# foolwood/SiamMask

Hardware: NVIDIA H100
Metric: search-region frames/sec (127/255 SiamMask-sharp) (higher is better)
Workload: dtype f16x3 (hi+lo split fp16 operands on wgmma, f32 accumulate; f32 CUDA-core xcorr/refine)

## Files before the change

### siammask_b200/csrc/common.cuh

```cuda
#pragma once
#include <cuda.h>
#include <cuda_fp16.h>
#include <cuda_runtime.h>
#include <cstdint>
#include <cstdio>
#include <stdexcept>
#include <string>
#include <vector>

namespace smk {

struct Act {
  __half* hi = nullptr;
  __half* lo = nullptr;
  int B = 0, H = 0, W = 0, C = 0;
  int sexp = 0;
  __host__ __device__ size_t numel() const { return (size_t)B * H * W * C; }
  __host__ __device__ int M() const { return B * H * W; }
};

struct ConvGeom {
  int Cin, Cout, KH, KW, stride, pad, dil;
  __host__ __device__ int out_size(int in) const { return (in + 2 * pad - dil * (KH - 1) - 1) / stride + 1; }
};

enum OutMode : int { OUT_NHWC_SPLIT = 0, OUT_NHWC_F32 = 1, OUT_NCHW_F32 = 2 };

struct Epilogue {
  const float* alpha = nullptr;
  const float* beta = nullptr;
  const __half* res_hi = nullptr;
  const __half* res_lo = nullptr;
  __half* out_hi = nullptr;
  __half* out_lo = nullptr;
  float* out_f32 = nullptr;
  int out_mode = OUT_NHWC_SPLIT;
  int relu = 0;
  int* ovf = nullptr;
};

__device__ __forceinline__ void flag_if_out_of_range(float absmax, int* ovf) {
  if (ovf != nullptr && !(absmax <= 65504.f)) atomicOr(ovf, 1);
}

struct GemmSegment {
  CUtensorMap tmA[2];
  int kind;
  int mode;
  int num_kb, cblks, KW;
  int stride, pad, dil;
  int b_col0;
};

struct GemmParams {
  GemmSegment seg[2];
  int nseg;
  CUtensorMap tmB[2];
  int M, Cout, Ho, Wo;
  int n_tiles, m_tiles;
  int reverse_m;
  Epilogue ep;
};

struct GemmInput {
  Act in;
  ConvGeom g;
  int w_col0;
};

struct TrackerHp {
  double context_amount, penalty_k, window_influence, lr;
  int32_t exemplar_size, instance_size, total_stride, base_size, out_size, reserved;
};

struct CudaError : std::runtime_error {
  using std::runtime_error::runtime_error;
};

#define SMK_CUDA(expr)                                                                              \
  do {                                                                                              \
    cudaError_t _e = (expr);                                                                        \
    if (_e != cudaSuccess)                                                                          \
      throw smk::CudaError(std::string(#expr) + " failed: " + cudaGetErrorString(_e) + " at " +    \
                           __FILE__ + ":" + std::to_string(__LINE__));                              \
  } while (0)

#define SMK_CHECK(cond, msg)                                                                        \
  do {                                                                                              \
    if (!(cond)) throw std::runtime_error(std::string("check failed: ") + #cond + " — " + (msg));   \
  } while (0)

template <typename K>
inline void ensure_dynamic_smem(K kernel, int bytes, unsigned long long& done_mask) {
  int dev = 0;
  SMK_CUDA(cudaGetDevice(&dev));
  const unsigned long long bit = 1ull << (dev & 63);
  if (done_mask & bit) return;
  SMK_CUDA(cudaFuncSetAttribute(kernel, cudaFuncAttributeMaxDynamicSharedMemorySize, bytes));
  done_mask |= bit;
}


bool gemm_conv_supported(const ConvGeom& g);
void launch_gemm_conv(const Act& in, const ConvGeom& g, const __half* w_hi, const __half* w_lo, int cout_pad,
                      const Epilogue& ep, int nsplit, int num_sms, cudaStream_t st);
void launch_gemm_multi(const GemmInput* convs, int nconv, const Act* residual, int res_col0, const __half* w_hi,
                       const __half* w_lo, int cout_pad, int w_ld, const Epilogue& ep, int nsplit, int num_sms,
                       cudaStream_t st, bool reverse_m = false);

CUtensorMap make_map_tiled_nd(const __half* base, int rank, const uint64_t* dims, const uint64_t* strides_bytes,
                              const uint32_t* box, int swizzle_bytes);

int patch_conv_mode();
// ... 47 lines not shown
```

### siammask_b200/csrc/conv_gemm_sm90.cu

```cuda
#include "common.cuh"
#include "ptx.cuh"

#include <cstdlib>
#include <cstring>
#include <mutex>
#include <unordered_map>

namespace smk {

namespace {

constexpr int BLOCK_M = 128;
constexpr int BLOCK_K = 64;
constexpr int CIN_GRAIN = 64;
constexpr int MMA_K = 16;
constexpr int SMEM_LIMIT = 227 * 1024;
constexpr int NUM_CONSUMER_WARPS = 8;
constexpr int NUM_THREADS = 128 + 32 * NUM_CONSUMER_WARPS;
constexpr int PRODUCER_REGS = 40;
constexpr int CONSUMER_REGS = 232;

template <int BLOCK_N, int NSPLIT>
struct Cfg {
  static constexpr int A_TILE_BYTES = BLOCK_M * BLOCK_K * 2;
  static constexpr int B_TILE_BYTES = BLOCK_N * BLOCK_K * 2;
  static constexpr int STAGE_BYTES = NSPLIT * (A_TILE_BYTES + B_TILE_BYTES);
  static constexpr int RAW_STAGES = (SMEM_LIMIT - 2048) / STAGE_BYTES;
  static constexpr int STAGES = RAW_STAGES > 6 ? 6 : RAW_STAGES;
  static constexpr int SMEM_BYTES = STAGES * STAGE_BYTES + 1024  + 256 ;
  static constexpr int ACC = BLOCK_N / 2;
  static_assert(STAGES >= 2, "pipeline needs at least two stages");
  static_assert(BLOCK_N % 16 == 0 && BLOCK_N >= 16 && BLOCK_N <= 128, "N tile (register accumulators)");
  static_assert(B_TILE_BYTES % 1024 == 0, "stage parts stay 1024-aligned (swizzle atoms)");
  static_assert(SMEM_BYTES <= SMEM_LIMIT, "shared memory budget");
};

__device__ __forceinline__ int m_block(const GemmParams& p, int tile) {
  const int mb = tile / p.n_tiles;
  return p.reverse_m ? p.m_tiles - 1 - mb : mb;
}

template <int BLOCK_N, int NSPLIT>
__global__ void __launch_bounds__(NUM_THREADS, 1) conv_gemm_kernel(const __grid_constant__ GemmParams p) {
  using C = Cfg<BLOCK_N, NSPLIT>;
  constexpr int STAGES = C::STAGES;
  constexpr int A_TILE_BYTES = C::A_TILE_BYTES;

  extern __shared__ uint8_t smem_raw[];
  uint8_t* smem = reinterpret_cast<uint8_t*>((reinterpret_cast<uintptr_t>(smem_raw) + 1023) & ~uintptr_t(1023));
  uint64_t* full_bar = reinterpret_cast<uint64_t*>(smem + STAGES * C::STAGE_BYTES);
  uint64_t* empty_bar = full_bar + STAGES;

  const int warp = __shfl_sync(0xffffffffu, (int)(threadIdx.x >> 5), 0);
  const int lane = threadIdx.x & 31;
  const int num_tiles = p.m_tiles * p.n_tiles;

  if (threadIdx.x == 0) {
    for (int i = 0; i < NSPLIT; ++i) {
      for (int sgi = 0; sgi < p.nseg; ++sgi) tma_prefetch_desc(&p.seg[sgi].tmA[i]);
      tma_prefetch_desc(&p.tmB[i]);
    }
    for (int s = 0; s < STAGES; ++s) {
      mbar_init(&full_bar[s], 1);
      mbar_init(&empty_bar[s], NUM_CONSUMER_WARPS);
    }
    fence_barrier_init();
  }
  __syncthreads();

  if (warp < 4) {
    setmaxnreg_dec<PRODUCER_REGS>();
    if (warp != 0) return;
    const bool leader = elect_one();
    int stage = 0;
    uint32_t phase = 0;
    auto acquire = [&](uint32_t bytes) {
      mbar_wait(&empty_bar[stage], phase ^ 1);
      if (leader) mbar_arrive_expect_tx(&full_bar[stage], bytes);
    };
    auto load_2d = [&](void* dst, const CUtensorMap* map, int c0, int c1) {
      if (leader) tma_load_2d(dst, map, &full_bar[stage], c0, c1);
    };
    for (int tile = blockIdx.x; tile < num_tiles; tile += gridDim.x) {
      const int m0 = m_block(p, tile) * BLOCK_M;
      const int n0 = (tile % p.n_tiles) * BLOCK_N;
      const int q = m0 % p.Wo;
      const int t = m0 / p.Wo;
      const int pq = t % p.Ho;
      const int nb = t / p.Ho;
      for (int sgi = 0; sgi < p.nseg; ++sgi) {
        const GemmSegment& sg = p.seg[sgi];
        if (sg.kind == 1) {
#pragma unroll 1
          for (int kb = 0; kb < BLOCK_N / BLOCK_K; ++kb) {
            acquire(C::STAGE_BYTES);
            uint8_t* st = smem + stage * C::STAGE_BYTES;
#pragma unroll
            for (int s = 0; s < NSPLIT; ++s) {
              load_2d(st + s * A_TILE_BYTES, &sg.tmA[s], n0 + kb * BLOCK_K, m0);
              load_2d(st + NSPLIT * A_TILE_BYTES + s * C::B_TILE_BYTES, &p.tmB[s], sg.b_col0 + n0 + kb * BLOCK_K, n0);
            }
            __syncwarp();
            if (++stage == STAGES) { stage = 0; phase ^= 1; }
          }
          continue;
        }
        const int wb = q * sg.stride - sg.pad;
        const int hb = pq * sg.stride - sg.pad;
#pragma unroll 1
        for (int kb = 0; kb < sg.num_kb; ++kb) {
          acquire(C::STAGE_BYTES);
          uint8_t* st = smem + stage * C::STAGE_BYTES;
          const int tap = kb / sg.cblks;
          const int c0 = (kb - tap * sg.cblks) * BLOCK_K;
#pragma unroll
          for (int s = 0; s < NSPLIT; ++s) {
            uint8_t* a_dst = st + s * A_TILE_BYTES;
            if (sg.mode == 0) {
              load_2d(a_dst, &sg.tmA[s], c0, m0);
            } else if (leader) {
              const int r = tap / sg.KW;
              const int sx = tap - r * sg.KW;
              tma_load_im2col_4d(a_dst, &sg.tmA[s], &full_bar[stage], c0, wb, hb, nb,
                                 static_cast<uint16_t>(sx * sg.dil), static_cast<uint16_t>(r * sg.dil));
            }
            load_2d(st + NSPLIT * A_TILE_BYTES + s * C::B_TILE_BYTES, &p.tmB[s], sg.b_col0 + kb * BLOCK_K, n0);
          }
          __syncwarp();
          if (++stage == STAGES) { stage = 0; phase ^= 1; }
        }
      }
    }
    return;
  }

  setmaxnreg_inc<CONSUMER_REGS>();
  const int wg = (warp >> 2) - 1;
  const int wl = warp & 3;
  const Epilogue& ep = p.ep;
  const int HoWo = p.Ho * p.Wo;
  float acc[C::ACC];
  float acc2[C::ACC];
  int stage = 0;
  uint32_t phase = 0;
  for (int tile = blockIdx.x; tile < num_tiles; tile += gridDim.x) {
#pragma unroll
    for (int i = 0; i < C::ACC; ++i) { acc[i] = 0.f; acc2[i] = 0.f; }
    int prev = -1;
    for (int sgi = 0; sgi < p.nseg; ++sgi) {
      const GemmSegment& sg = p.seg[sgi];
      const bool ident = sg.kind == 1;
      const int nkb = ident ? BLOCK_N / BLOCK_K : sg.num_kb;
#pragma unroll 1
      for (int kb = 0; kb < nkb; ++kb) {
        mbar_wait(&full_bar[stage], phase);
        const uint32_t a_hi = smem_u32(smem + stage * C::STAGE_BYTES) + wg * (64 * BLOCK_K * 2);
        const uint32_t b_hi = smem_u32(smem + stage * C::STAGE_BYTES) + NSPLIT * A_TILE_BYTES;
        const uint64_t da_hi0 = wgmma_desc_kmajor<128>(a_hi);
        const uint64_t db_hi0 = wgmma_desc_kmajor<128>(b_hi);
        const uint64_t da_lo0 = wgmma_desc_kmajor<128>(a_hi + A_TILE_BYTES);
        const uint64_t db_lo0 = wgmma_desc_kmajor<128>(b_hi + C::B_TILE_BYTES);
        wgmma_fence();
#pragma unroll
        for (int k = 0; k < BLOCK_K / MMA_K; ++k) {
          const uint64_t kadd = static_cast<uint64_t>(k * MMA_K * 2 / 16);
          wgmma_f16<BLOCK_N>(acc, da_hi0 + kadd, db_hi0 + kadd);
          if constexpr (NSPLIT == 2) {
            wgmma_f16<BLOCK_N>(acc2, da_hi0 + kadd, db_lo0 + kadd);
            wgmma_f16<BLOCK_N>(acc2, da_lo0 + kadd, db_hi0 + kadd);
          }
        }
        wgmma_commit();
        wgmma_wait<1>();
        if (prev >= 0) {
          __syncwarp();
          if (lane == 0) mbar_arrive(&empty_bar[prev]);
        }
        prev = stage;
        if (++stage == STAGES) { stage = 0; phase ^= 1; }
      }
    }
    wgmma_wait<0>();
    fence_regs(acc);
    if constexpr (NSPLIT == 2) fence_regs(acc2);
    __syncwarp();
    if (lane == 0) mbar_arrive(&empty_bar[prev]);

    const int row0 = m_block(p, tile) * BLOCK_M + wg * 64 + wl * 16 + (lane >> 2);
    const int col0 = (tile % p.n_tiles) * BLOCK_N + 2 * (lane & 3);
    float amax = 0.f;
#pragma unroll
    for (int h = 0; h < 2; ++h) {
      const int m = row0 + 8 * h;
      if (m >= p.M) continue;
      const int b = m / HoWo;
      const int hw = m - b * HoWo;
#pragma unroll
      for (int j = 0; j < BLOCK_N / 8; ++j) {
        const int n = col0 + 8 * j;
        float v0 = acc[4 * j + 2 * h], v1 = acc[4 * j + 2 * h + 1];
        if constexpr (NSPLIT == 2) {
          v0 += acc2[4 * j + 2 * h];
          v1 += acc2[4 * j + 2 * h + 1];
        }
        const float2 al = __ldg(reinterpret_cast<const float2*>(ep.alpha + n));
        const float2 be = __ldg(reinterpret_cast<const float2*>(ep.beta + n));
        v0 = fmaf(v0, al.x, be.x);
        v1 = fmaf(v1, al.y, be.y);
        const size_t off = static_cast<size_t>(m) * p.Cout + n;
        if (ep.res_hi != nullptr) {
          const float2 f = __half22float2(*reinterpret_cast<const __half2*>(ep.res_hi + off));
          v0 += f.x;
          v1 += f.y;
          if (ep.res_lo != nullptr) {
            const float2 l = __half22float2(*reinterpret_cast<const __half2*>(ep.res_lo + off));
            v0 += l.x;
            v1 += l.y;
          }
        }
        if (ep.relu) {
          v0 = fmaxf(v0, 0.f);
          v1 = fmaxf(v1, 0.f);
        }
        if (ep.out_mode == OUT_NHWC_SPLIT) {
          amax = fmaxf(amax, fmaxf(fabsf(v0), fabsf(v1)));
          const __half2 hv = __floats2half2_rn(v0, v1);
          const float2 hf = __half22float2(hv);
          *reinterpret_cast<__half2*>(ep.out_hi + off) = hv;
          if (ep.out_lo != nullptr)
            *reinterpret_cast<__half2*>(ep.out_lo + off) = __floats2half2_rn(v0 - hf.x, v1 - hf.y);
        } else if (ep.out_mode == OUT_NHWC_F32) {
          *reinterpret_cast<float2*>(ep.out_f32 + off) = make_float2(v0, v1);
        } else if (n < p.Cout) {
          float* dst = ep.out_f32 + (static_cast<size_t>(b) * p.Cout + n) * HoWo + hw;
          __stcs(dst, v0);
          if (n + 1 < p.Cout) __stcs(dst + HoWo, v1);
        }
      }
    }
    if (ep.out_mode == OUT_NHWC_SPLIT) flag_if_out_of_range(amax, ep.ovf);
  }
}

using EncodeTiledFn = CUresult (*)(CUtensorMap*, CUtensorMapDataType, cuuint32_t, void*, const cuuint64_t*,
                                   const cuuint64_t*, const cuuint32_t*, const cuuint32_t*, CUtensorMapInterleave,
                                   CUtensorMapSwizzle, CUtensorMapL2promotion, CUtensorMapFloatOOBfill);
using EncodeIm2colFn = CUresult (*)(CUtensorMap*, CUtensorMapDataType, cuuint32_t, void*, const cuuint64_t*,
                                    const cuuint64_t*, const int*, const int*, cuuint32_t, cuuint32_t,
                                    const cuuint32_t*, CUtensorMapInterleave, CUtensorMapSwizzle,
                                    CUtensorMapL2promotion, CUtensorMapFloatOOBfill);

struct DriverApi {
  EncodeTiledFn tiled = nullptr;
  EncodeIm2colFn im2col = nullptr;
  int driver_version = 0;
};

const DriverApi& driver_api() {
  static DriverApi api;
  static std::once_flag once;
  std::call_once(once, [] {
    void* fn = nullptr;
    cudaDriverEntryPointQueryResult q;
    SMK_CUDA(cudaGetDriverEntryPoint("cuTensorMapEncodeTiled", &fn, cudaEnableDefault, &q));
    SMK_CHECK(fn != nullptr && q == cudaDriverEntryPointSuccess, "cuTensorMapEncodeTiled not available");
    api.tiled = reinterpret_cast<EncodeTiledFn>(fn);
    fn = nullptr;
    SMK_CUDA(cudaGetDriverEntryPoint("cuTensorMapEncodeIm2col", &fn, cudaEnableDefault, &q));
    SMK_CHECK(fn != nullptr && q == cudaDriverEntryPointSuccess, "cuTensorMapEncodeIm2col not available");
    api.im2col = reinterpret_cast<EncodeIm2colFn>(fn);
    SMK_CUDA(cudaDriverGetVersion(&api.driver_version));
  });
  return api;
}

struct MapKey {
  uint64_t v[16];
  bool operator==(const MapKey& o) const { return std::memcmp(v, o.v, sizeof v) == 0; }
};
struct MapKeyHash {
  size_t operator()(const MapKey& k) const {
    uint64_t h = 0x9E3779B97F4A7C15ull;
    for (uint64_t x : k.v) { h ^= x + 0x9E3779B97F4A7C15ull + (h << 6) + (h >> 2); }
    return (size_t)h;
  }
};
template <typename F>
CUtensorMap cached_map(const MapKey& key, F&& encode) {
  static std::mutex mu;
  static std::unordered_map<MapKey, CUtensorMap, MapKeyHash> cache;
  static const bool off = getenv("SMB200_NO_MAP_CACHE") != nullptr;
  if (off) return encode();
  int dev = 0;
  cudaGetDevice(&dev);
  MapKey k = key;
  k.v[15] = (uint64_t)dev;
  std::lock_guard<std::mutex> lock(mu);
  auto it = cache.find(k);
  if (it != cache.end()) return it->second;
  if (cache.size() > 65536) cache.clear();
  CUtensorMap m = encode();
  cache.emplace(k, m);
  return m;
}

CUtensorMap make_map_2d_raw(const __half* base, uint64_t inner, uint64_t outer, uint32_t box_inner, uint32_t box_outer) {
  CUtensorMap m;
  cuuint64_t dims[2] = {inner, outer};
  cuuint64_t strides[1] = {inner * sizeof(__half)};
  cuuint32_t box[2] = {box_inner, box_outer};
  cuuint32_t estr[2] = {1, 1};
  const CUtensorMapSwizzle sw = box_inner == 64 ? CU_TENSOR_MAP_SWIZZLE_128B : CU_TENSOR_MAP_SWIZZLE_64B;
  CUresult r = driver_api().tiled(&m, CU_TENSOR_MAP_DATA_TYPE_FLOAT16, 2, const_cast<__half*>(base), dims, strides,
                                  box, estr, CU_TENSOR_MAP_INTERLEAVE_NONE, sw,
                                  CU_TENSOR_MAP_L2_PROMOTION_L2_256B, CU_TENSOR_MAP_FLOAT_OOB_FILL_NONE);
  SMK_CHECK(r == CUDA_SUCCESS, "cuTensorMapEncodeTiled failed, code " + std::to_string((int)r));
  return m;
}

CUtensorMap make_map_2d(const __half* base, uint64_t inner, uint64_t outer, uint32_t box_inner, uint32_t box_outer) {
  MapKey k{};
  k.v[0] = 1; k.v[1] = (uint64_t)base; k.v[2] = inner; k.v[3] = outer; k.v[4] = box_inner; k.v[5] = box_outer;
  return cached_map(k, [&] { return make_map_2d_raw(base, inner, outer, box_inner, box_outer); });
}

CUtensorMap make_map_im2col_raw(const __half* base, const Act& in, const ConvGeom& g, int bk) {
  CUtensorMap m;
  cuuint64_t dims[4] = {(cuuint64_t)in.C, (cuuint64_t)in.W, (cuuint64_t)in.H, (cuuint64_t)in.B};
  cuuint64_t strides[3] = {(cuuint64_t)in.C * 2, (cuuint64_t)in.W * in.C * 2, (cuuint64_t)in.H * in.W * in.C * 2};
  int lower[2] = {-g.pad, -g.pad};
  int upper[2] = {g.pad - (g.KW - 1) * g.dil, g.pad - (g.KH - 1) * g.dil};
  cuuint32_t estr[4] = {1, (cuuint32_t)g.stride, (cuuint32_t)g.stride, 1};
  const DriverApi& api = driver_api();
  CUresult r = api.im2col(&m, CU_TENSOR_MAP_DATA_TYPE_FLOAT16, 4, const_cast<__half*>(base), dims, strides, lower,
                          upper, bk, BLOCK_M, estr, CU_TENSOR_MAP_INTERLEAVE_NONE,
                          bk == 64 ? CU_TENSOR_MAP_SWIZZLE_128B : CU_TENSOR_MAP_SWIZZLE_64B,
                          CU_TENSOR_MAP_L2_PROMOTION_L2_256B, CU_TENSOR_MAP_FLOAT_OOB_FILL_NONE);
  SMK_CHECK(r == CUDA_SUCCESS, "cuTensorMapEncodeIm2col failed, code " + std::to_string((int)r));
  if (api.driver_version <= 13010 && in.numel() * sizeof(__half) < 131072)
    reinterpret_cast<uint64_t*>(&m)[1] &= ~(1ull << 21);
  return m;
}

CUtensorMap make_map_im2col(const __half* base, const Act& in, const ConvGeom& g, int bk) {
  MapKey k{};
  k.v[0] = 3; k.v[1] = (uint64_t)base;
  k.v[2] = ((uint64_t)in.B << 32) | (uint32_t)in.H; k.v[3] = ((uint64_t)in.W << 32) | (uint32_t)in.C;
  k.v[4] = ((uint64_t)g.KH << 32) | (uint32_t)g.KW; k.v[5] = ((uint64_t)g.stride << 32) | (uint32_t)g.pad;
  k.v[6] = ((uint64_t)g.dil << 32) | (uint32_t)bk;
  return cached_map(k, [&] { return make_map_im2col_raw(base, in, g, bk); });
}

template <int BLOCK_N, int NSPLIT>
void launch_cfg(const GemmParams& p, int num_sms, cudaStream_t st) {
  using C = Cfg<BLOCK_N, NSPLIT>;
  auto kern = conv_gemm_kernel<BLOCK_N, NSPLIT>;
  static unsigned long long attr_done = 0;
  ensure_dynamic_smem(kern, C::SMEM_BYTES, attr_done);
  const int tiles = p.m_tiles * p.n_tiles;
  const int grid = tiles < num_sms ? tiles : num_sms;
  kern<<<grid, NUM_THREADS, C::SMEM_BYTES, st>>>(p);
  SMK_CUDA(cudaGetLastError());
}

}

static CUtensorMap make_map_2d_any_raw(const __half* base, uint64_t inner, uint64_t outer, uint32_t box_inner, uint32_t box_outer,
                            int swizzle_bytes) {
  CUtensorMap m;
  cuuint64_t dims[2] = {inner, outer};
  cuuint64_t strides[1] = {inner * sizeof(__half)};
  cuuint32_t box[2] = {box_inner, box_outer};
  cuuint32_t estr[2] = {1, 1};
  const CUtensorMapSwizzle sw = swizzle_bytes == 128 ? CU_TENSOR_MAP_SWIZZLE_128B
                                : swizzle_bytes == 64 ? CU_TENSOR_MAP_SWIZZLE_64B : CU_TENSOR_MAP_SWIZZLE_32B;
  CUresult r = driver_api().tiled(&m, CU_TENSOR_MAP_DATA_TYPE_FLOAT16, 2, const_cast<__half*>(base), dims, strides,
                                  box, estr, CU_TENSOR_MAP_INTERLEAVE_NONE, sw, CU_TENSOR_MAP_L2_PROMOTION_L2_128B,
                                  CU_TENSOR_MAP_FLOAT_OOB_FILL_NONE);
  SMK_CHECK(r == CUDA_SUCCESS, "cuTensorMapEncodeTiled failed, code " + std::to_string((int)r));
  return m;
}

CUtensorMap make_map_2d_any(const __half* base, uint64_t inner, uint64_t outer, uint32_t box_inner, uint32_t box_outer,
                            int swizzle_bytes) {
  MapKey k{};
  k.v[0] = 5; k.v[1] = (uint64_t)base; k.v[2] = inner; k.v[3] = outer; k.v[4] = box_inner; k.v[5] = box_outer;
  k.v[6] = (uint64_t)swizzle_bytes;
  return cached_map(k, [&] { return make_map_2d_any_raw(base, inner, outer, box_inner, box_outer, swizzle_bytes); });
}

static CUtensorMap make_map_tiled_nd_raw(const __half* base, int rank, const uint64_t* dims,
                                         const uint64_t* strides_bytes, const uint32_t* box, int swizzle_bytes) {
  SMK_CHECK(rank >= 2 && rank <= 5, "tensor map rank");
  CUtensorMap m;
  cuuint64_t d[5], sb[4];
  cuuint32_t bx[5], es[5];
  for (int i = 0; i < rank; ++i) { d[i] = dims[i]; bx[i] = box[i]; es[i] = 1; }
  for (int i = 0; i + 1 < rank; ++i) sb[i] = strides_bytes[i];
  const CUtensorMapSwizzle sw = swizzle_bytes == 128 ? CU_TENSOR_MAP_SWIZZLE_128B
                                : swizzle_bytes == 64 ? CU_TENSOR_MAP_SWIZZLE_64B
                                : swizzle_bytes == 32 ? CU_TENSOR_MAP_SWIZZLE_32B : CU_TENSOR_MAP_SWIZZLE_NONE;
  CUresult r = driver_api().tiled(&m, CU_TENSOR_MAP_DATA_TYPE_FLOAT16, (cuuint32_t)rank, const_cast<__half*>(base), d, sb,
                                  bx, es, CU_TENSOR_MAP_INTERLEAVE_NONE, sw, CU_TENSOR_MAP_L2_PROMOTION_L2_256B,
                                  CU_TENSOR_MAP_FLOAT_OOB_FILL_NONE);
  SMK_CHECK(r == CUDA_SUCCESS, "cuTensorMapEncodeTiled (nd) failed, code " + std::to_string((int)r));
  return m;
}

CUtensorMap make_map_tiled_nd(const __half* base, int rank, const uint64_t* dims, const uint64_t* strides_bytes,
                              const uint32_t* box, int swizzle_bytes) {
  SMK_CHECK(rank >= 2 && rank <= 5, "tensor map rank");
  MapKey k{};
  k.v[0] = 4 | ((uint64_t)rank << 8) | ((uint64_t)swizzle_bytes << 16);
  k.v[1] = (uint64_t)base;
  for (int i = 0; i < rank; ++i) k.v[2 + i] = dims[i] | ((uint64_t)box[i] << 40);
  for (int i = 0; i + 1 < rank; ++i) k.v[7 + i] = strides_bytes[i];
  return cached_map(k, [&] { return make_map_tiled_nd_raw(base, rank, dims, strides_bytes, box, swizzle_bytes); });
}

bool gemm_conv_supported(const ConvGeom& g) { return g.Cin % CIN_GRAIN == 0 && g.Cout >= 1; }

int gemm_cout_pad(int cout) {
  if (cout <= 16) return 16;
  if (cout <= 32) return 32;
  if (cout <= 64) return 64;
  if (cout <= 128) return 128;
  return (cout + 255) / 256 * 256;
}

void launch_gemm_conv(const Act& in, const ConvGeom& g, const __half* w_hi, const __half* w_lo, int cout_pad,
                      const Epilogue& ep, int nsplit, int num_sms, cudaStream_t st) {
  GemmInput gi{in, g, 0};
  launch_gemm_multi(&gi, 1, nullptr, -1, w_hi, w_lo, cout_pad, g.KH * g.KW * g.Cin, ep, nsplit, num_sms, st);
}

void launch_gemm_multi(const GemmInput* convs, int nconv, const Act* residual, int res_col0, const __half* w_hi,
                       const __half* w_lo, int cout_pad, int w_ld, const Epilogue& ep_in, int nsplit, int num_sms,
                       cudaStream_t st, bool reverse_m) {
  SMK_CHECK(nconv >= 1 && nconv <= 2, "1 or 2 convolution segments");
  SMK_CHECK(nconv + (residual != nullptr ? 1 : 0) <= 2, "at most two K segments");
  Epilogue ep = ep_in;
  const ConvGeom& g0 = convs[0].g;
  const Act& in0 = convs[0].in;
  const int Ho = g0.out_size(in0.H), Wo = g0.out_size(in0.W);
  GemmParams p;
  p.M = in0.B * Ho * Wo;
  p.Cout = g0.Cout;
  p.Ho = Ho;
  p.Wo = Wo;
  const int block_n = cout_pad < 128 ? cout_pad : 128;
  const int bk = BLOCK_K;
  SMK_CHECK(cout_pad % block_n == 0, "cout_pad must be a multiple of the N tile");
  if (ep.out_mode != OUT_NCHW_F32) SMK_CHECK(g0.Cout == cout_pad, "NHWC outputs need Cout to match the padded tile width");
  p.n_tiles = cout_pad / block_n;
  p.m_tiles = (p.M + BLOCK_M - 1) / BLOCK_M;
  p.reverse_m = reverse_m ? 1 : 0;
  p.nseg = 0;
  for (int i = 0; i < nconv; ++i) {
    const ConvGeom& g = convs[i].g;
    const Act& in = convs[i].in;
    SMK_CHECK(gemm_conv_supported(g), "Cin must be a multiple of 64 for the tensor-core conv");
    SMK_CHECK(in.C == g.Cin && g.Cout == g0.Cout && in.B == in0.B, "segment channels/batch mismatch");
    SMK_CHECK(g.out_size(in.H) == Ho && g.out_size(in.W) == Wo, "segments must produce the same output size");
    SMK_CHECK(nsplit == 1 || (in.lo != nullptr && w_lo != nullptr), "exact mode needs lo planes");
    GemmSegment& sg = p.seg[p.nseg++];
    sg.kind = 0;
    sg.cblks = g.Cin / bk;
    sg.num_kb = g.KH * g.KW * sg.cblks;
    sg.KW = g.KW;
    sg.stride = g.stride;
    sg.pad = g.pad;
    sg.dil = g.dil;
    sg.mode = (g.KH == 1 && g.KW == 1 && g.stride == 1 && g.pad == 0) ? 0 : 1;
    sg.b_col0 = convs[i].w_col0;
    SMK_CHECK(sg.b_col0 % 64 == 0 && sg.b_col0 + g.KH * g.KW * g.Cin <= w_ld, "weight column range");
    for (int s = 0; s < nsplit; ++s) {
      const __half* a = s == 0 ? in.hi : in.lo;
      sg.tmA[s] = sg.mode == 0 ? make_map_2d(a, g.Cin, (uint64_t)in.M(), bk, BLOCK_M) : make_map_im2col(a, in, g, bk);
    }
    if (nsplit == 1) sg.tmA[1] = sg.tmA[0];
  }
  if (residual != nullptr) {
    SMK_CHECK(res_col0 >= 0 && res_col0 % 64 == 0 && res_col0 + g0.Cout <= w_ld && block_n % 64 == 0,
              "identity segment needs a diagonal block in the packed weights");
    SMK_CHECK(residual->C == g0.Cout && residual->M() == p.M, "residual shape");
    SMK_CHECK(nsplit == 1 || residual->lo != nullptr, "exact mode residual needs both planes");
    GemmSegment& sg = p.seg[p.nseg++];
    sg.kind = 1;
    sg.mode = 0;
    sg.num_kb = block_n / bk;
    sg.cblks = sg.KW = sg.stride = sg.dil = 1;
    sg.pad = 0;
    sg.b_col0 = res_col0;
    for (int s = 0; s < nsplit; ++s)
      sg.tmA[s] = make_map_2d(s == 0 ? residual->hi : residual->lo, g0.Cout, (uint64_t)p.M, bk, BLOCK_M);
    if (nsplit == 1) sg.tmA[1] = sg.tmA[0];
    ep.res_hi = ep.res_lo = nullptr;
  }
  if (p.nseg == 1) p.seg[1] = p.seg[0];
  for (int s = 0; s < nsplit; ++s)
    p.tmB[s] = make_map_2d(s == 0 ? w_hi : w_lo, (uint64_t)w_ld, cout_pad, bk, block_n);
  if (nsplit == 1) p.tmB[1] = p.tmB[0];
  p.ep = ep;

#define SMK_DISPATCH(BN)                                             \
  case BN:                                                           \
    if (nsplit == 2) launch_cfg<BN, 2>(p, num_sms, st);              \
    else launch_cfg<BN, 1>(p, num_sms, st);                          \
    break;
  switch (block_n) {
    SMK_DISPATCH(16)
    SMK_DISPATCH(32)
    SMK_DISPATCH(64)
    SMK_DISPATCH(128)
    default: SMK_CHECK(false, "unsupported N tile");
  }
#undef SMK_DISPATCH
}

}
```

### siammask_b200/csrc/ptx.cuh

```cuda
#pragma once
#include <cstdint>
#include <cuda.h>

namespace smk {

__device__ __forceinline__ uint32_t smem_u32(const void* p) {
  return static_cast<uint32_t>(__cvta_generic_to_shared(p));
}

__device__ __forceinline__ bool elect_one() {
  uint32_t pred;
  asm volatile(
      "{\n\t.reg .pred p;\n\t"
      "elect.sync _|p, 0xffffffff;\n\t"
      "selp.u32 %0, 1, 0, p;\n\t}\n"
      : "=r"(pred));
  return pred != 0;
}

__device__ __forceinline__ void mbar_init(uint64_t* bar, uint32_t count) {
  asm volatile("mbarrier.init.shared::cta.b64 [%0], %1;" ::"r"(smem_u32(bar)), "r"(count) : "memory");
}
__device__ __forceinline__ void fence_barrier_init() {
  asm volatile("fence.mbarrier_init.release.cluster;" ::: "memory");
}
__device__ __forceinline__ void fence_proxy_async() {
  asm volatile("fence.proxy.async.shared::cta;" ::: "memory");
}
__device__ __forceinline__ void mbar_arrive_expect_tx(uint64_t* bar, uint32_t bytes) {
  asm volatile("mbarrier.arrive.expect_tx.shared::cta.b64 _, [%0], %1;" ::"r"(smem_u32(bar)), "r"(bytes)
               : "memory");
}
__device__ __forceinline__ void mbar_arrive(uint64_t* bar) {
  asm volatile("mbarrier.arrive.shared::cta.b64 _, [%0];" ::"r"(smem_u32(bar)) : "memory");
}
__device__ __forceinline__ void mbar_wait(uint64_t* bar, uint32_t parity) {
  asm volatile(
      "{\n\t.reg .pred p;\n\t"
      "WAIT_%=:\n\t"
      "mbarrier.try_wait.parity.shared::cta.b64 p, [%0], %1;\n\t"
      "@p bra DONE_%=;\n\t"
      "bra WAIT_%=;\n\t"
      "DONE_%=:\n\t}\n" ::"r"(smem_u32(bar)),
      "r"(parity)
      : "memory");
}

__device__ __forceinline__ void tma_prefetch_desc(const CUtensorMap* m) {
  asm volatile("prefetch.tensormap [%0];" ::"l"(reinterpret_cast<uint64_t>(m)) : "memory");
}
__device__ __forceinline__ void tma_load_2d(void* dst, const CUtensorMap* map, uint64_t* bar, int c0, int c1) {
  asm volatile(
      "cp.async.bulk.tensor.2d.shared::cluster.global.mbarrier::complete_tx::bytes"
      " [%0], [%1, {%3, %4}], [%2];" ::"r"(smem_u32(dst)),
      "l"(reinterpret_cast<uint64_t>(map)), "r"(smem_u32(bar)), "r"(c0), "r"(c1)
      : "memory");
}
__device__ __forceinline__ void tma_load_im2col_4d(void* dst, const CUtensorMap* map, uint64_t* bar, int c, int w,
                                                   int h, int n, uint16_t off_w, uint16_t off_h) {
  asm volatile(
      "cp.async.bulk.tensor.4d.shared::cluster.global.im2col.mbarrier::complete_tx::bytes"
      " [%0], [%1, {%3, %4, %5, %6}], [%2], {%7, %8};" ::"r"(smem_u32(dst)),
      "l"(reinterpret_cast<uint64_t>(map)), "r"(smem_u32(bar)), "r"(c), "r"(w), "r"(h), "r"(n), "h"(off_w),
      "h"(off_h)
      : "memory");
}

__device__ __forceinline__ void tma_store_2d(const CUtensorMap* map, const void* src, int c0, int c1) {
  asm volatile("cp.async.bulk.tensor.2d.global.shared::cta.bulk_group [%0, {%2, %3}], [%1];" ::"l"(
                   reinterpret_cast<uint64_t>(map)),
               "r"(smem_u32(src)), "r"(c0), "r"(c1)
               : "memory");
}
__device__ __forceinline__ void tma_store_commit() { asm volatile("cp.async.bulk.commit_group;" ::: "memory"); }
template <int N>
__device__ __forceinline__ void tma_store_wait_read() {
  asm volatile("cp.async.bulk.wait_group.read %0;" ::"n"(N) : "memory");
}
__device__ __forceinline__ void tma_store_wait_all() { asm volatile("cp.async.bulk.wait_group 0;" ::: "memory"); }

template <int SW>
__device__ __forceinline__ uint64_t wgmma_desc_kmajor(uint32_t smem_addr) {
  static_assert(SW == 128 || SW == 64, "swizzle span");
  uint64_t d = 0;
  d |= static_cast<uint64_t>((smem_addr & 0x3FFFF) >> 4);
  d |= static_cast<uint64_t>(1) << 16;
  d |= static_cast<uint64_t>((8 * SW) >> 4) << 32;
  d |= static_cast<uint64_t>(SW == 128 ? 1 : 2) << 62;
  return d;
}
__device__ __forceinline__ void wgmma_fence() { asm volatile("wgmma.fence.sync.aligned;" ::: "memory"); }
__device__ __forceinline__ void wgmma_commit() { asm volatile("wgmma.commit_group.sync.aligned;" ::: "memory"); }
template <int N>
__device__ __forceinline__ void wgmma_wait() { asm volatile("wgmma.wait_group.sync.aligned %0;" ::"n"(N) : "memory"); }
template <int R>
__device__ __forceinline__ void fence_regs(float (&d)[R]) {
#pragma unroll
  for (int i = 0; i < R; ++i) asm volatile("" : "+f"(d[i])::"memory");
}
template <int RDEC>
__device__ __forceinline__ void setmaxnreg_dec() { asm volatile("setmaxnreg.dec.sync.aligned.u32 %0;" ::"n"(RDEC)); }
template <int RINC>
__device__ __forceinline__ void setmaxnreg_inc() { asm volatile("setmaxnreg.inc.sync.aligned.u32 %0;" ::"n"(RINC)); }

template <int N>
__device__ __forceinline__ void wgmma_f16(float (&d)[N / 2], uint64_t da, uint64_t db);
template <>
__device__ __forceinline__ void wgmma_f16<16>(float (&d)[8], uint64_t da, uint64_t db) {
  asm volatile(
      "{\n\t.reg .pred p;\n\tsetp.ne.b32 p, %10, 0;\n\t"
      "wgmma.mma_async.sync.aligned.m64n16k16.f32.f16.f16 "
      "{%0, %1, %2, %3, %4, %5, %6, %7}, %8, %9, p, 1, 1, 0, 0;\n\t}\n"
      : "+f"(d[0]), "+f"(d[1]), "+f"(d[2]), "+f"(d[3]), "+f"(d[4]), "+f"(d[5]), "+f"(d[6]), "+f"(d[7])
      : "l"(da), "l"(db), "r"(1));
}
template <>
__device__ __forceinline__ void wgmma_f16<32>(float (&d)[16], uint64_t da, uint64_t db) {
  asm volatile(
// ... 38 lines not shown
```

Measured before the change: 3774.

## Use thread-block clusters with TMA multicast to share A/B tiles in conv GEMM

Launches the conv GEMM with 2-CTA clusters, shaped by K depth, so neighbouring CTAs split and multicast shared A or B operand tiles via TMA. Each CTA loads a slice and multicasts it, and empty-barrier releases are sent across the cluster with mapa and remote arrive. This targets L2/global load traffic for deep-K layers. In exchange it adds cross-CTA synchronisation, cluster scheduling limits on occupancy, and padded M tiles for odd tile counts.

After: 3793, median of 6. No clear change (+0.5%).

```diff
diff --git a/siammask_b200/csrc/common.cuh b/siammask_b200/csrc/common.cuh
--- a/siammask_b200/csrc/common.cuh
+++ b/siammask_b200/csrc/common.cuh
@@ -59,6 +59,7 @@
   int M, Cout, Ho, Wo;
   int n_tiles, m_tiles;
   int reverse_m;
+  int cm, cn;
   Epilogue ep;
 };
 
diff --git a/siammask_b200/csrc/conv_gemm_sm90.cu b/siammask_b200/csrc/conv_gemm_sm90.cu
--- a/siammask_b200/csrc/conv_gemm_sm90.cu
+++ b/siammask_b200/csrc/conv_gemm_sm90.cu
@@ -1,6 +1,7 @@
 #include "common.cuh"
 #include "ptx.cuh"
 
+#include <cstdio>
 #include <cstdlib>
 #include <cstring>
 #include <mutex>
@@ -35,9 +36,11 @@
   static_assert(SMEM_BYTES <= SMEM_LIMIT, "shared memory budget");
 };
 
-__device__ __forceinline__ int m_block(const GemmParams& p, int tile) {
-  const int mb = tile / p.n_tiles;
-  return p.reverse_m ? p.m_tiles - 1 - mb : mb;
+__device__ __forceinline__ int2 group_tile(const GemmParams& p, int g, int rm, int rn) {
+  const int n_groups = p.n_tiles / p.cn;
+  const int m_groups = (p.m_tiles + p.cm - 1) / p.cm;
+  const int gm = g / n_groups;
+  return make_int2((p.reverse_m ? m_groups - 1 - gm : gm) * p.cm + rm, (g - gm * n_groups) * p.cn + rn);
 }
 
 template <int BLOCK_N, int NSPLIT>
@@ -53,7 +56,11 @@
 
   const int warp = __shfl_sync(0xffffffffu, (int)(threadIdx.x >> 5), 0);
   const int lane = threadIdx.x & 31;
-  const int num_tiles = p.m_tiles * p.n_tiles;
+  const int cm = p.cm, cn = p.cn;
+  const int rank = static_cast<int>(cluster_ctarank());
+  const int rm = rank / cn, rn = rank - (rank / cn) * cn;
+  const int num_groups = (p.m_tiles + cm - 1) / cm * (p.n_tiles / cn);
+  const int num_clusters = gridDim.x / (cm * cn);
 
   if (threadIdx.x == 0) {
     for (int i = 0; i < NSPLIT; ++i) {
@@ -62,184 +69,203 @@
     }
     for (int s = 0; s < STAGES; ++s) {
       mbar_init(&full_bar[s], 1);
-      mbar_init(&empty_bar[s], NUM_CONSUMER_WARPS);
+      mbar_init(&empty_bar[s], NUM_CONSUMER_WARPS * (cm + cn - 1));
     }
     fence_barrier_init();
   }
-  __syncthreads();
+  if (cm * cn > 1) cluster_sync();
+  else __syncthreads();
 
   if (warp < 4) {
     setmaxnreg_dec<PRODUCER_REGS>();
-    if (warp != 0) return;
-    const bool leader = elect_one();
-    int stage = 0;
-    uint32_t phase = 0;
-    auto acquire = [&](uint32_t bytes) {
-      mbar_wait(&empty_bar[stage], phase ^ 1);
-      if (leader) mbar_arrive_expect_tx(&full_bar[stage], bytes);
-    };
-    auto load_2d = [&](void* dst, const CUtensorMap* map, int c0, int c1) {
-      if (leader) tma_load_2d(dst, map, &full_bar[stage], c0, c1);
-    };
-    for (int tile = blockIdx.x; tile < num_tiles; tile += gridDim.x) {
-      const int m0 = m_block(p, tile) * BLOCK_M;
-      const int n0 = (tile % p.n_tiles) * BLOCK_N;
-      const int q = m0 % p.Wo;
-      const int t = m0 / p.Wo;
-      const int pq = t % p.Ho;
-      const int nb = t / p.Ho;
-      for (int sgi = 0; sgi < p.nseg; ++sgi) {
-        const GemmSegment& sg = p.seg[sgi];
-        if (sg.kind == 1) {
+    if (warp == 0) {
+      const bool leader = elect_one();
+      const uint16_t a_mask = static_cast<uint16_t>(((1u << cn) - 1) << (rm * cn));
+      const uint16_t b_mask = static_cast<uint16_t>((cm == 2 ? 1u | (1u << cn) : 1u) << rn);
+      const int a_rows = BLOCK_M / cn;
+      const int b_rows = BLOCK_N / cm;
+      int stage = 0;
+      uint32_t phase = 0;
+      auto acquire = [&](uint32_t bytes) {
+        mbar_wait(&empty_bar[stage], phase ^ 1);
+        if (leader) mbar_arrive_expect_tx(&full_bar[stage], bytes);
+      };
+      auto load_2d = [&](void* dst, const CUtensorMap* map, int c0, int c1, uint16_t mask) {
+        if (!leader) return;
+        if (mask == (1u << rank)) tma_load_2d(dst, map, &full_bar[stage], c0, c1);
+        else tma_load_2d_mc(dst, map, &full_bar[stage], c0, c1, mask);
+      };
+      for (int g = blockIdx.x / (cm * cn); g < num_groups; g += num_clusters) {
+        const int2 tile = group_tile(p, g, rm, rn);
+        const int m0 = min(tile.x, p.m_tiles - 1) * BLOCK_M;
+        const int n0 = tile.y * BLOCK_N;
+        const int ma = min(m0 + rn * a_rows, p.M - 1);
+        const int q = ma % p.Wo;
+        const int t = ma / p.Wo;
+        const int pq = t % p.Ho;
+        const int nb = t / p.Ho;
+        for (int sgi = 0; sgi < p.nseg; ++sgi) {
+          const GemmSegment& sg = p.seg[sgi];
+          if (sg.kind == 1) {
 #pragma unroll 1
-          for (int kb = 0; kb < BLOCK_N / BLOCK_K; ++kb) {
+            for (int kb = 0; kb < BLOCK_N / BLOCK_K; ++kb) {
+              acquire(C::STAGE_BYTES);
+              uint8_t* st = smem + stage * C::STAGE_BYTES;
+#pragma unroll
+              for (int s = 0; s < NSPLIT; ++s) {
+                load_2d(st + s * A_TILE_BYTES, &sg.tmA[s], n0 + kb * BLOCK_K, m0, 1u << rank);
+                load_2d(st + NSPLIT * A_TILE_BYTES + s * C::B_TILE_BYTES + rm * (C::B_TILE_BYTES / cm), &p.tmB[s],
+                        sg.b_col0 + n0 + kb * BLOCK_K, n0 + rm * b_rows, b_mask);
+              }
+              __syncwarp();
+              if (++stage == STAGES) { stage = 0; phase ^= 1; }
+            }
+            continue;
+          }
+          const int wb = q * sg.stride - sg.pad;
+          const int hb = pq * sg.stride - sg.pad;
+#pragma unroll 1
+          for (int kb = 0; kb < sg.num_kb; ++kb) {
             acquire(C::STAGE_BYTES);
             uint8_t* st = smem + stage * C::STAGE_BYTES;
+            const int tap = kb / sg.cblks;
+            const int c0 = (kb - tap * sg.cblks) * BLOCK_K;
 #pragma unroll
             for (int s = 0; s < NSPLIT; ++s) {
-              load_2d(st + s * A_TILE_BYTES, &sg.tmA[s], n0 + kb * BLOCK_K, m0);
-              load_2d(st + NSPLIT * A_TILE_BYTES + s * C::B_TILE_BYTES, &p.tmB[s], sg.b_col0 + n0 + kb * BLOCK_K, n0);
+              uint8_t* a_dst = st + s * A_TILE_BYTES + rn * (A_TILE_BYTES / cn);
+              if (sg.mode == 0) {
+                load_2d(a_dst, &sg.tmA[s], c0, ma, a_mask);
+              } else if (leader) {
+                const int r = tap / sg.KW;
+                const int sx = tap - r * sg.KW;
+                const uint16_t ow = static_cast<uint16_t>(sx * sg.dil), oh = static_cast<uint16_t>(r * sg.dil);
+                if (cn == 1) tma_load_im2col_4d(a_dst, &sg.tmA[s], &full_bar[stage], c0, wb, hb, nb, ow, oh);
+                else tma_load_im2col_4d_mc(a_dst, &sg.tmA[s], &full_bar[stage], c0, wb, hb, nb, ow, oh, a_mask);
+              }
+              load_2d(st + NSPLIT * A_TILE_BYTES + s * C::B_TILE_BYTES + rm * (C::B_TILE_BYTES / cm), &p.tmB[s],
+                      sg.b_col0 + kb * BLOCK_K, n0 + rm * b_rows, b_mask);
             }
             __syncwarp();
             if (++stage == STAGES) { stage = 0; phase ^= 1; }
           }
-          continue;
         }
-        const int wb = q * sg.stride - sg.pad;
-        const int hb = pq * sg.stride - sg.pad;
+      }
+    }
+  } else {
+    setmaxnreg_inc<CONSUMER_REGS>();
+    const int wg = (warp >> 2) - 1;
+    const int wl = warp & 3;
+    const Epilogue& ep = p.ep;
+    const int HoWo = p.Ho * p.Wo;
+    int peer = -1;
+    if (lane < cm) peer = lane * cn + rn;
+    else if (lane < cm + cn - 1) peer = rm * cn + (lane - cm < rn ? lane - cm : lane - cm + 1);
+    const uint32_t peer_empty = peer >= 0 ? mapa_shared(smem_u32(empty_bar), static_cast<uint32_t>(peer)) : 0u;
+    auto release = [&](int s) {
+      __syncwarp();
+      if (peer >= 0) mbar_arrive_cluster(peer_empty + s * static_cast<uint32_t>(sizeof(uint64_t)));
+    };
+    float acc[C::ACC];
+    float acc2[C::ACC];
+    int stage = 0;
+    uint32_t phase = 0;
+    for (int g = blockIdx.x / (cm * cn); g < num_groups; g += num_clusters) {
+      const int2 tile = group_tile(p, g, rm, rn);
+#pragma unroll
+      for (int i = 0; i < C::ACC; ++i) { acc[i] = 0.f; acc2[i] = 0.f; }
+      int prev = -1;
+      for (int sgi = 0; sgi < p.nseg; ++sgi) {
+        const GemmSegment& sg = p.seg[sgi];
+        const bool ident = sg.kind == 1;
+        const int nkb = ident ? BLOCK_N / BLOCK_K : sg.num_kb;
 #pragma unroll 1
-        for (int kb = 0; kb < sg.num_kb; ++kb) {
-          acquire(C::STAGE_BYTES);
-          uint8_t* st = smem + stage * C::STAGE_BYTES;
-          const int tap = kb / sg.cblks;
-          const int c0 = (kb - tap * sg.cblks) * BLOCK_K;
+        for (int kb = 0; kb < nkb; ++kb) {
+          mbar_wait(&full_bar[stage], phase);
+          const uint32_t a_hi = smem_u32(smem + stage * C::STAGE_BYTES) + wg * (64 * BLOCK_K * 2);
+          const uint32_t b_hi = smem_u32(smem + stage * C::STAGE_BYTES) + NSPLIT * A_TILE_BYTES;
+          const uint64_t da_hi0 = wgmma_desc_kmajor<128>(a_hi);
+          const uint64_t db_hi0 = wgmma_desc_kmajor<128>(b_hi);
+          const uint64_t da_lo0 = wgmma_desc_kmajor<128>(a_hi + A_TILE_BYTES);
+          const uint64_t db_lo0 = wgmma_desc_kmajor<128>(b_hi + C::B_TILE_BYTES);
+          wgmma_fence();
 #pragma unroll
-          for (int s = 0; s < NSPLIT; ++s) {
-            uint8_t* a_dst = st + s * A_TILE_BYTES;
-            if (sg.mode == 0) {
-              load_2d(a_dst, &sg.tmA[s], c0, m0);
-            } else if (leader) {
-              const int r = tap / sg.KW;
-              const int sx = tap - r * sg.KW;
-              tma_load_im2col_4d(a_dst, &sg.tmA[s], &full_bar[stage], c0, wb, hb, nb,
-                                 static_cast<uint16_t>(sx * sg.dil), static_cast<uint16_t>(r * sg.dil));
+          for (int k = 0; k < BLOCK_K / MMA_K; ++k) {
+            const uint64_t kadd = static_cast<uint64_t>(k * MMA_K * 2 / 16);
+            wgmma_f16<BLOCK_N>(acc, da_hi0 + kadd, db_hi0 + kadd);
+            if constexpr (NSPLIT == 2) {
+              wgmma_f16<BLOCK_N>(acc2, da_hi0 + kadd, db_lo0 + kadd);
+              wgmma_f16<BLOCK_N>(acc2, da_lo0 + kadd, db_hi0 + kadd);
             }
-            load_2d(st + NSPLIT * A_TILE_BYTES + s * C::B_TILE_BYTES, &p.tmB[s], sg.b_col0 + kb * BLOCK_K, n0);
-          }
-          __syncwarp();
+          }
+          wgmma_commit();
+          wgmma_wait<1>();
+          if (prev >= 0) release(prev);
+          prev = stage;
           if (++stage == STAGES) { stage = 0; phase ^= 1; }
         }
       }
-    }
-    return;
-  }
-
-  setmaxnreg_inc<CONSUMER_REGS>();
-  const int wg = (warp >> 2) - 1;
-  const int wl = warp & 3;
-  const Epilogue& ep = p.ep;
-  const int HoWo = p.Ho * p.Wo;
-  float acc[C::ACC];
-  float acc2[C::ACC];
-  int stage = 0;
-  uint32_t phase = 0;
-  for (int tile = blockIdx.x; tile < num_tiles; tile += gridDim.x) {
+      wgmma_wait<0>();
+      fence_regs(acc);
+      if constexpr (NSPLIT == 2) fence_regs(acc2);
+      release(prev);
+      if (tile.x >= p.m_tiles) continue;
+
+      const int row0 = tile.x * BLOCK_M + wg * 64 + wl * 16 + (lane >> 2);
+      const int col0 = tile.y * BLOCK_N + 2 * (lane & 3);
+      float amax = 0.f;
 #pragma unroll
-    for (int i = 0; i < C::ACC; ++i) { acc[i] = 0.f; acc2[i] = 0.f; }
-    int prev = -1;
-    for (int sgi = 0; sgi < p.nseg; ++sgi) {
-      const GemmSegment& sg = p.seg[sgi];
-      const bool ident = sg.kind == 1;
-      const int nkb = ident ? BLOCK_N / BLOCK_K : sg.num_kb;
-#pragma unroll 1
-      for (int kb = 0; kb < nkb; ++kb) {
-        mbar_wait(&full_bar[stage], phase);
-        const uint32_t a_hi = smem_u32(smem + stage * C::STAGE_BYTES) + wg * (64 * BLOCK_K * 2);
-        const uint32_t b_hi = smem_u32(smem + stage * C::STAGE_BYTES) + NSPLIT * A_TILE_BYTES;
-        const uint64_t da_hi0 = wgmma_desc_kmajor<128>(a_hi);
-        const uint64_t db_hi0 = wgmma_desc_kmajor<128>(b_hi);
-        const uint64_t da_lo0 = wgmma_desc_kmajor<128>(a_hi + A_TILE_BYTES);
-        const uint64_t db_lo0 = wgmma_desc_kmajor<128>(b_hi + C::B_TILE_BYTES);
-        wgmma_fence();
+      for (int h = 0; h < 2; ++h) {
+        const int m = row0 + 8 * h;
+        if (m >= p.M) continue;
+        const int b = m / HoWo;
+        const int hw = m - b * HoWo;
 #pragma unroll
-        for (int k = 0; k < BLOCK_K / MMA_K; ++k) {
-          const uint64_t kadd = static_cast<uint64_t>(k * MMA_K * 2 / 16);
-          wgmma_f16<BLOCK_N>(acc, da_hi0 + kadd, db_hi0 + kadd);
+        for (int j = 0; j < BLOCK_N / 8; ++j) {
+          const int n = col0 + 8 * j;
+          float v0 = acc[4 * j + 2 * h], v1 = acc[4 * j + 2 * h + 1];
           if constexpr (NSPLIT == 2) {
-            wgmma_f16<BLOCK_N>(acc2, da_hi0 + kadd, db_lo0 + kadd);
-            wgmma_f16<BLOCK_N>(acc2, da_lo0 + kadd, db_hi0 + kadd);
-          }
-        }
-        wgmma_commit();
-        wgmma_wait<1>();
-        if (prev >= 0) {
-          __syncwarp();
-          if (lane == 0) mbar_arrive(&empty_bar[prev]);
-        }
-        prev = stage;
-        if (++stage == STAGES) { stage = 0; phase ^= 1; }
-      }
-    }
-    wgmma_wait<0>();
-    fence_regs(acc);
-    if constexpr (NSPLIT == 2) fence_regs(acc2);
-    __syncwarp();
-    if (lane == 0) mbar_arrive(&empty_bar[prev]);
-
-    const int row0 = m_block(p, tile) * BLOCK_M + wg * 64 + wl * 16 + (lane >> 2);
-    const int col0 = (tile % p.n_tiles) * BLOCK_N + 2 * (lane & 3);
-    float amax = 0.f;
-#pragma unroll
-    for (int h = 0; h < 2; ++h) {
-      const int m = row0 + 8 * h;
-      if (m >= p.M) continue;
-      const int b = m / HoWo;
-      const int hw = m - b * HoWo;
-#pragma unroll
-      for (int j = 0; j < BLOCK_N / 8; ++j) {
-        const int n = col0 + 8 * j;
-        float v0 = acc[4 * j + 2 * h], v1 = acc[4 * j + 2 * h + 1];
-        if constexpr (NSPLIT == 2) {
-          v0 += acc2[4 * j + 2 * h];
-          v1 += acc2[4 * j + 2 * h + 1];
-        }
-        const float2 al = __ldg(reinterpret_cast<const float2*>(ep.alpha + n));
-        const float2 be = __ldg(reinterpret_cast<const float2*>(ep.beta + n));
-        v0 = fmaf(v0, al.x, be.x);
-        v1 = fmaf(v1, al.y, be.y);
-        const size_t off = static_cast<size_t>(m) * p.Cout + n;
-        if (ep.res_hi != nullptr) {
-          const float2 f = __half22float2(*reinterpret_cast<const __half2*>(ep.res_hi + off));
-          v0 += f.x;
-          v1 += f.y;
-          if (ep.res_lo != nullptr) {
-            const float2 l = __half22float2(*reinterpret_cast<const __half2*>(ep.res_lo + off));
-            v0 += l.x;
-            v1 += l.y;
-          }
-        }
-        if (ep.relu) {
-          v0 = fmaxf(v0, 0.f);
-          v1 = fmaxf(v1, 0.f);
-        }
-        if (ep.out_mode == OUT_NHWC_SPLIT) {
-          amax = fmaxf(amax, fmaxf(fabsf(v0), fabsf(v1)));
-          const __half2 hv = __floats2half2_rn(v0, v1);
-          const float2 hf = __half22float2(hv);
-          *reinterpret_cast<__half2*>(ep.out_hi + off) = hv;
-          if (ep.out_lo != nullptr)
-            *reinterpret_cast<__half2*>(ep.out_lo + off) = __floats2half2_rn(v0 - hf.x, v1 - hf.y);
-        } else if (ep.out_mode == OUT_NHWC_F32) {
-          *reinterpret_cast<float2*>(ep.out_f32 + off) = make_float2(v0, v1);
-        } else if (n < p.Cout) {
-          float* dst = ep.out_f32 + (static_cast<size_t>(b) * p.Cout + n) * HoWo + hw;
-          __stcs(dst, v0);
-          if (n + 1 < p.Cout) __stcs(dst + HoWo, v1);
+            v0 += acc2[4 * j + 2 * h];
+            v1 += acc2[4 * j + 2 * h + 1];
+          }
+          const float2 al = __ldg(reinterpret_cast<const float2*>(ep.alpha + n));
+          const float2 be = __ldg(reinterpret_cast<const float2*>(ep.beta + n));
+          v0 = fmaf(v0, al.x, be.x);
+          v1 = fmaf(v1, al.y, be.y);
+          const size_t off = static_cast<size_t>(m) * p.Cout + n;
+          if (ep.res_hi != nullptr) {
+            const float2 f = __half22float2(*reinterpret_cast<const __half2*>(ep.res_hi + off));
+            v0 += f.x;
+            v1 += f.y;
+            if (ep.res_lo != nullptr) {
+              const float2 l = __half22float2(*reinterpret_cast<const __half2*>(ep.res_lo + off));
+              v0 += l.x;
+              v1 += l.y;
+            }
+          }
+          if (ep.relu) {
+            v0 = fmaxf(v0, 0.f);
+            v1 = fmaxf(v1, 0.f);
+          }
+          if (ep.out_mode == OUT_NHWC_SPLIT) {
+            amax = fmaxf(amax, fmaxf(fabsf(v0), fabsf(v1)));
+            const __half2 hv = __floats2half2_rn(v0, v1);
+            const float2 hf = __half22float2(hv);
+            *reinterpret_cast<__half2*>(ep.out_hi + off) = hv;
+            if (ep.out_lo != nullptr)
+              *reinterpret_cast<__half2*>(ep.out_lo + off) = __floats2half2_rn(v0 - hf.x, v1 - hf.y);
+          } else if (ep.out_mode == OUT_NHWC_F32) {
+            *reinterpret_cast<float2*>(ep.out_f32 + off) = make_float2(v0, v1);
+          } else if (n < p.Cout) {
+            float* dst = ep.out_f32 + (static_cast<size_t>(b) * p.Cout + n) * HoWo + hw;
+            __stcs(dst, v0);
+            if (n + 1 < p.Cout) __stcs(dst + HoWo, v1);
+          }
         }
       }
+      if (ep.out_mode == OUT_NHWC_SPLIT) flag_if_out_of_range(amax, ep.ovf);
     }
-    if (ep.out_mode == OUT_NHWC_SPLIT) flag_if_out_of_range(amax, ep.ovf);
-  }
+  }
+  if (cm * cn > 1) cluster_sync();
 }
 
 using EncodeTiledFn = CUresult (*)(CUtensorMap*, CUtensorMapDataType, cuuint32_t, void*, const cuuint64_t*,
@@ -324,7 +350,7 @@
   return cached_map(k, [&] { return make_map_2d_raw(base, inner, outer, box_inner, box_outer); });
 }
 
-CUtensorMap make_map_im2col_raw(const __half* base, const Act& in, const ConvGeom& g, int bk) {
+CUtensorMap make_map_im2col_raw(const __half* base, const Act& in, const ConvGeom& g, int bk, int pixels) {
   CUtensorMap m;
   cuuint64_t dims[4] = {(cuuint64_t)in.C, (cuuint64_t)in.W, (cuuint64_t)in.H, (cuuint64_t)in.B};
   cuuint64_t strides[3] = {(cuuint64_t)in.C * 2, (cuuint64_t)in.W * in.C * 2, (cuuint64_t)in.H * in.W * in.C * 2};
@@ -333,7 +359,7 @@
   cuuint32_t estr[4] = {1, (cuuint32_t)g.stride, (cuuint32_t)g.stride, 1};
   const DriverApi& api = driver_api();
   CUresult r = api.im2col(&m, CU_TENSOR_MAP_DATA_TYPE_FLOAT16, 4, const_cast<__half*>(base), dims, strides, lower,
-                          upper, bk, BLOCK_M, estr, CU_TENSOR_MAP_INTERLEAVE_NONE,
+                          upper, bk, pixels, estr, CU_TENSOR_MAP_INTERLEAVE_NONE,
                           bk == 64 ? CU_TENSOR_MAP_SWIZZLE_128B : CU_TENSOR_MAP_SWIZZLE_64B,
                           CU_TENSOR_MAP_L2_PROMOTION_L2_256B, CU_TENSOR_MAP_FLOAT_OOB_FILL_NONE);
   SMK_CHECK(r == CUDA_SUCCESS, "cuTensorMapEncodeIm2col failed, code " + std::to_string((int)r));
@@ -342,13 +368,34 @@
   return m;
 }
 
-CUtensorMap make_map_im2col(const __half* base, const Act& in, const ConvGeom& g, int bk) {
+CUtensorMap make_map_im2col(const __half* base, const Act& in, const ConvGeom& g, int bk, int pixels) {
   MapKey k{};
   k.v[0] = 3; k.v[1] = (uint64_t)base;
   k.v[2] = ((uint64_t)in.B << 32) | (uint32_t)in.H; k.v[3] = ((uint64_t)in.W << 32) | (uint32_t)in.C;
   k.v[4] = ((uint64_t)g.KH << 32) | (uint32_t)g.KW; k.v[5] = ((uint64_t)g.stride << 32) | (uint32_t)g.pad;
-  k.v[6] = ((uint64_t)g.dil << 32) | (uint32_t)bk;
-  return cached_map(k, [&] { return make_map_im2col_raw(base, in, g, bk); });
+  k.v[6] = ((uint64_t)g.dil << 32) | (uint32_t)bk; k.v[7] = (uint64_t)pixels;
+  return cached_map(k, [&] { return make_map_im2col_raw(base, in, g, bk, pixels); });
+}
+
+constexpr int CLUSTER_MIN_KB = 32;
+void cluster_shape(int m_tiles, int n_tiles, int kb_per_tile, int& cm, int& cn) {
+  static const int forced = [] {
+    const char* e = std::getenv("SMB200_GEMM_CLUSTER");
+    if (e == nullptr) return 0;
+    int a = 0, b = 0;
+    char tail = 0;
+    SMK_CHECK(std::sscanf(e, "%dx%d%c", &a, &b, &tail) == 2 && (a == 1 || a == 2) && (b == 1 || b == 2),
+              "SMB200_GEMM_CLUSTER must be 1x1, 1x2, 2x1 or 2x2");
+    return 10 * a + b;
+  }();
+  if (forced != 0) {
+    cm = m_tiles >= 2 ? forced / 10 : 1;
+    cn = n_tiles % 2 == 0 ? forced % 10 : 1;
+  } else {
+    const bool share = kb_per_tile >= CLUSTER_MIN_KB;
+    cn = share && n_tiles % 2 == 0 ? 2 : 1;
+    cm = share && cn == 1 && m_tiles >= 2 ? 2 : 1;
+  }
 }
 
 template <int BLOCK_N, int NSPLIT>
@@ -357,10 +404,34 @@
   auto kern = conv_gemm_kernel<BLOCK_N, NSPLIT>;
   static unsigned long long attr_done = 0;
   ensure_dynamic_smem(kern, C::SMEM_BYTES, attr_done);
-  const int tiles = p.m_tiles * p.n_tiles;
-  const int grid = tiles < num_sms ? tiles : num_sms;
-  kern<<<grid, NUM_THREADS, C::SMEM_BYTES, st>>>(p);
-  SMK_CUDA(cudaGetLastError());
+  const int csize = p.cm * p.cn;
+  const int groups = (p.m_tiles + p.cm - 1) / p.cm * (p.n_tiles / p.cn);
+  cudaLaunchAttribute attr;
+  attr.id = cudaLaunchAttributeClusterDimension;
+  attr.val.clusterDim.x = csize;
+  attr.val.clusterDim.y = 1;
+  attr.val.clusterDim.z = 1;
+  cudaLaunchConfig_t cfg = {};
+  cfg.blockDim = dim3(NUM_THREADS);
+  cfg.dynamicSmemBytes = C::SMEM_BYTES;
+  cfg.stream = st;
+  int clusters = num_sms;
+  if (csize > 1) {
+    cfg.attrs = &attr;
+    cfg.numAttrs = 1;
+    cfg.gridDim = dim3(csize);
+    static int resident[64][2] = {};
+    int dev = 0;
+    SMK_CUDA(cudaGetDevice(&dev));
+    int& fit = resident[dev & 63][csize / 4];
+    if (fit == 0) SMK_CUDA(cudaOccupancyMaxActiveClusters(&fit, kern, &cfg));
+    SMK_CHECK(fit > 0, "conv_gemm_kernel: no cluster of this size fits on the device");
+    if (fit < clusters / csize) clusters = fit;
+    else clusters /= csize;
+  }
+  const int grid = groups < clusters ? groups : clusters;
+  cfg.gridDim = dim3(grid * csize);
+  SMK_CUDA(cudaLaunchKernelEx(&cfg, kern, p));
 }
 
 }
@@ -455,6 +526,9 @@
   p.n_tiles = cout_pad / block_n;
   p.m_tiles = (p.M + BLOCK_M - 1) / BLOCK_M;
   p.reverse_m = reverse_m ? 1 : 0;
+  int kb_per_tile = residual != nullptr ? block_n / bk : 0;
+  for (int i = 0; i < nconv; ++i) kb_per_tile += convs[i].g.KH * convs[i].g.KW * (convs[i].g.Cin / bk);
+  cluster_shape(p.m_tiles, p.n_tiles, kb_per_tile, p.cm, p.cn);
   p.nseg = 0;
   for (int i = 0; i < nconv; ++i) {
     const ConvGeom& g = convs[i].g;
@@ -476,7 +550,8 @@
     SMK_CHECK(sg.b_col0 % 64 == 0 && sg.b_col0 + g.KH * g.KW * g.Cin <= w_ld, "weight column range");
     for (int s = 0; s < nsplit; ++s) {
       const __half* a = s == 0 ? in.hi : in.lo;
-      sg.tmA[s] = sg.mode == 0 ? make_map_2d(a, g.Cin, (uint64_t)in.M(), bk, BLOCK_M) : make_map_im2col(a, in, g, bk);
+      sg.tmA[s] = sg.mode == 0 ? make_map_2d(a, g.Cin, (uint64_t)in.M(), bk, BLOCK_M / p.cn)
+                               : make_map_im2col(a, in, g, bk, BLOCK_M / p.cn);
     }
     if (nsplit == 1) sg.tmA[1] = sg.tmA[0];
   }
@@ -499,7 +574,7 @@
   }
   if (p.nseg == 1) p.seg[1] = p.seg[0];
   for (int s = 0; s < nsplit; ++s)
-    p.tmB[s] = make_map_2d(s == 0 ? w_hi : w_lo, (uint64_t)w_ld, cout_pad, bk, block_n);
+    p.tmB[s] = make_map_2d(s == 0 ? w_hi : w_lo, (uint64_t)w_ld, cout_pad, bk, block_n / p.cm);
   if (nsplit == 1) p.tmB[1] = p.tmB[0];
   p.ep = ep;
 
diff --git a/siammask_b200/csrc/ptx.cuh b/siammask_b200/csrc/ptx.cuh
--- a/siammask_b200/csrc/ptx.cuh
+++ b/siammask_b200/csrc/ptx.cuh
@@ -64,6 +64,42 @@
       "l"(reinterpret_cast<uint64_t>(map)), "r"(smem_u32(bar)), "r"(c), "r"(w), "r"(h), "r"(n), "h"(off_w),
       "h"(off_h)
       : "memory");
+}
+
+__device__ __forceinline__ void tma_load_2d_mc(void* dst, const CUtensorMap* map, uint64_t* bar, int c0, int c1,
+                                               uint16_t cta_mask) {
+  asm volatile(
+      "cp.async.bulk.tensor.2d.shared::cluster.global.mbarrier::complete_tx::bytes.multicast::cluster"
+      " [%0], [%1, {%3, %4}], [%2], %5;" ::"r"(smem_u32(dst)),
+      "l"(reinterpret_cast<uint64_t>(map)), "r"(smem_u32(bar)), "r"(c0), "r"(c1), "h"(cta_mask)
+      : "memory");
+}
+__device__ __forceinline__ void tma_load_im2col_4d_mc(void* dst, const CUtensorMap* map, uint64_t* bar, int c, int w,
+                                                      int h, int n, uint16_t off_w, uint16_t off_h,
+                                                      uint16_t cta_mask) {
+  asm volatile(
+      "cp.async.bulk.tensor.4d.shared::cluster.global.im2col.mbarrier::complete_tx::bytes.multicast::cluster"
+      " [%0], [%1, {%3, %4, %5, %6}], [%2], {%7, %8}, %9;" ::"r"(smem_u32(dst)),
+      "l"(reinterpret_cast<uint64_t>(map)), "r"(smem_u32(bar)), "r"(c), "r"(w), "r"(h), "r"(n), "h"(off_w),
+      "h"(off_h), "h"(cta_mask)
+      : "memory");
+}
+
+__device__ __forceinline__ uint32_t cluster_ctarank() {
+  uint32_t r;
+  asm volatile("mov.u32 %0, %%cluster_ctarank;" : "=r"(r));
+  return r;
+}
+__device__ __forceinline__ uint32_t mapa_shared(uint32_t local, uint32_t rank) {
+  uint32_t r;
+  asm volatile("mapa.shared::cluster.u32 %0, %1, %2;" : "=r"(r) : "r"(local), "r"(rank));
+  return r;
+}
+__device__ __forceinline__ void mbar_arrive_cluster(uint32_t cluster_addr) {
+  asm volatile("mbarrier.arrive.shared::cluster.b64 _, [%0];" ::"r"(cluster_addr) : "memory");
+}
+__device__ __forceinline__ void cluster_sync() {
+  asm volatile("barrier.cluster.arrive.release;\n\tbarrier.cluster.wait.acquire;" ::: "memory");
 }
 
 __device__ __forceinline__ void tma_store_2d(const CUtensorMap* map, const void* src, int c0, int c1) {
```
